# Emieeel/auto_oo

Measured on AMD Instinct MI355X. Metric: OO-VQE energy+grad evals/sec (formaldimine CAS(4e,3o)/cc-pVDZ); 2e-transform fp64 TFLOP/s vs roofline, higher is better.
Workload: dtype f64; 1 GPU; configs[1] shape: N=43 AOs, n_occ=6, CAS(4e,3o), UCCD n_theta=4, n_kappa=327; one step = one batched call evaluating energy + full gradient of all 256 geometries of the rank (256 synthetic geometries in the job, geometry g on rank g mod n_gpus); value = evaluations/s; in-order calls on one stream; geometries_per_rank=256, batched_calls=1332, calls=in order, parallelism=geometry-sharded x1, one all_gather at the end, dist_world_size=1, devices_visible=1, device_of_rank0=0

## Files before the change

### auto_oo_amd/csrc/api.hip

```cpp
#include "common.h"
#include <stdarg.h>
#include <vector>
#include <utility>

static thread_local char g_err[512] = "";

void oovqe_set_error(const char* fmt, ...)
{
    va_list ap;
    va_start(ap, fmt);
    vsnprintf(g_err, sizeof(g_err), fmt, ap);
    va_end(ap);
}

extern "C" int oovqe_version(void) { return 100; }

extern "C" const char* oovqe_last_error(void) { return g_err; }

extern "C" int oovqe_device_count(void)
{
    int n = 0;
    hipError_t e = hipGetDeviceCount(&n);
    if (e != hipSuccess) {
        oovqe_set_error("hipGetDeviceCount: %s", hipGetErrorString(e));
        return -1;
    }
    return n;
}

#include <mutex>
#include <map>
int oovqe_ensure_dynamic_lds(const void* kernel, size_t bytes)
{
    static std::mutex mu;
    static std::map<std::pair<const void*, int>, size_t> done;
    int dev = 0;
    if (hipGetDevice(&dev) != hipSuccess) dev = 0;
    std::lock_guard<std::mutex> lock(mu);
    size_t& have = done[std::make_pair(kernel, dev)];
    if (bytes <= have) return 0;
    hipError_t e = hipFuncSetAttribute(kernel, hipFuncAttributeMaxDynamicSharedMemorySize, (int)bytes);
    if (e != hipSuccess) {
        oovqe_set_error("hipFuncSetAttribute(MaxDynamicSharedMemorySize = %zu): %s", bytes, hipGetErrorString(e));
        return OOVQE_ERR_HIP;
    }
    have = bytes;
    return 0;
}

static int g_opts[OOVQE_OPT_COUNT] = {0};
static const char* const g_opt_names[OOVQE_OPT_COUNT] = {
    "half_stream_old", "gm_two_per_cu", "gm_one_per_cu", "fused_chunks", "tri_plain_w", "cas_unfused",
    "sym_no_rs", "sym_mirror", "sym_simple", "sym_two_step", "no_ride", "tri_mode", "k1_no_pair", "k1_force_wide", "gm_plain_grid",
    "newton_one_wg", "sector_unfused", "sector_probe", "hess_vk_pass", "hess_own_stage1", "panel_rows",
    "k1_force_nt", "newton_no_chol", "tiles_variant", "sector_lambda_w", "sector_rdm_r3", "gm_three_per_cu", "panel_no_w",
    "stage1_free_run", "one_stream"};
static_assert(sizeof(g_opt_names) / sizeof(g_opt_names[0]) == OOVQE_OPT_COUNT, "option name table out of step with oovqe_option_t");

int oovqe_opt(int id) { return (id >= 0 && id < OOVQE_OPT_COUNT) ? g_opts[id] : 0; }

static char g_stage1[160] = "";
void oovqe_note_stage1(const char* fmt, ...)
{
    va_list ap;
    va_start(ap, fmt);
    vsnprintf(g_stage1, sizeof(g_stage1), fmt, ap);
    va_end(ap);
}
extern "C" const char* oovqe_last_stage1_kernel(void) { return g_stage1; }

extern "C" int oovqe_debug_set_option(const char* name, int value)
{
    for (int i = 0; name && i < OOVQE_OPT_COUNT; ++i)
        if (strcmp(name, g_opt_names[i]) == 0) { g_opts[i] = value; return 0; }
    oovqe_set_error("oovqe_debug_set_option: unknown option '%s'", name ? name : "(null)");
    return OOVQE_ERR_ARG;
}

extern "C" int oovqe_debug_get_option(const char* name)
{
    for (int i = 0; name && i < OOVQE_OPT_COUNT; ++i)
        if (strcmp(name, g_opt_names[i]) == 0) return g_opts[i];
    return -1;
}

namespace {
struct Internals {
    hipEvent_t ev[64] = {};
    hipStream_t st[1] = {nullptr};
    unsigned next = 0;
    bool tried = false, streams_tried = false;
};
Internals g_int[16];
std::mutex g_int_mu;

Internals* internals()
{
    int dev = 0;
    if (hipGetDevice(&dev) != hipSuccess || dev < 0 || dev >= 16) return nullptr;
    Internals& I = g_int[dev];
    if (!I.tried) {
        I.tried = true;
        for (int i = 0; i < 64; ++i)
            if (hipEventCreateWithFlags(&I.ev[i], hipEventDisableTiming) != hipSuccess) I.ev[i] = nullptr;
    }
    return &I;
}
}

hipEvent_t oovqe_internal_event()
{
    std::lock_guard<std::mutex> lock(g_int_mu);
    Internals* I = internals();
    return I ? I->ev[I->next++ & 63] : nullptr;
}

hipStream_t oovqe_internal_stream(int k)
{
    if (oovqe_opt(OOVQE_OPT_ONE_STREAM) != 0 || k != 0) return nullptr;
    std::lock_guard<std::mutex> lock(g_int_mu);
    Internals* I = internals();
    if (!I) return nullptr;
    if (!I->streams_tried) {
        I->streams_tried = true;
        if (hipStreamCreateWithFlags(&I->st[0], hipStreamNonBlocking) != hipSuccess) I->st[0] = nullptr;
    }
    return I->st[k];
}

static hipStream_t g_s1_stream[16];
static hipEvent_t g_s1_event[16];
static bool g_s1_seen[16];
static int g_s1_multi[16];

int oovqe_stage1_enter(hipStream_t st)
{
    int dev = 0;
    if (hipGetDevice(&dev) != hipSuccess || dev < 0 || dev >= 16) return 0;
    if (oovqe_opt(OOVQE_OPT_STAGE1_FREE_RUN) != 0) return 0;
// ... 123 lines not shown
```

### auto_oo_amd/csrc/cas.hip

```cpp
#include "common.h"
#include "circuit_small.h"
#include <type_traits>
#include <stdlib.h>

int oovqe_mode_contract_impl(const double* T, const double* Cm, double* out, long A, int K, int J,
                             long B, int ldc, int last, hipStream_t st);
int oovqe_mode_contract_batched(const double* T, const double* Cm, double* out, long A, int K, int J,
                                long B, int ldc, int last, int batch, long t_bs, long c_bs, long o_bs,
                                hipStream_t st);
int oovqe_mode_contract_batched_circ(const double* T, const double* Cm, double* out, long A, int K, int J,
                                     long B, int ldc, int last, int batch, long t_bs, long c_bs,
                                     long o_bs, hipStream_t st, const oovqe_circuit_job_t* cj);
int oovqe_contract_hosts_circuit(long A, int K, int J, long B, int last, int batch);
int oovqe_circuit_rdms_w(const double* theta, int n_theta, const oovqe_gate_t* gates, int n_gates, int n_qubits,
                         int ncas, uint32_t init_index, int want_tangents, int batch, double* psi, double* dpsi,
                         double* gamma, double* Gamma, double* work, const double* h_ao, const double* C, int N,
                         double* Wpre, oovqe_stream_t stream);
extern "C" int oovqe_circuit_rdms(const double* theta, int n_theta, const oovqe_gate_t* gates, int n_gates,
                                  int n_qubits, int ncas, uint32_t init_index, int want_tangents, int batch,
                                  double* psi, double* dpsi, double* gamma, double* Gamma, double* work,
                                  oovqe_stream_t stream);
extern "C" int oovqe_circuit_rdms_is_small(int n_qubits, int ncas, int nvec, int n_gates);

namespace {
// ... 2655 lines not shown
    }
    for (int o = 32; o > 0; o >>= 1) part += __shfl_xor(part, o);
    if ((tid & 63) == 0) red[tid >> 6] = part;
    __syncthreads();
    if (tid == 0) Epart[(size_t)k * N + n] = (red[0] + red[1]) + (red[2] + red[3]);
    if (k == 0) {
        if (tid == 0) Cpart[n] = n < no ? hmo[(size_t)n * M + n] + FIn[n] : 0.0;
        if (n >= no && n < M) {
            const int p = n - no;
            for (int q = tid; q < na; q += FROW_THREADS) c1[p * na + q] = FIn[no + q];
            for (int idx = tid; idx < na3; idx += FROW_THREADS) c2[(size_t)p * na3 + idx] = 0.5 * cube[idx];
        }
    }
}

__global__ __launch_bounds__(512)
void cas_final_kernel(const double* __restrict__ Fcol, const double* __restrict__ Epart,
                      const double* __restrict__ Cpart, double nuc, int nrdm, int N, int M,
                      const int32_t* __restrict__ kap_row, const int32_t* __restrict__ kap_col,
                      int n_kappa, double* __restrict__ c0, double* __restrict__ E,
                      double* __restrict__ gvec, double* __restrict__ dE, double* __restrict__ fock,
                      double* __restrict__ gmat, const double* __restrict__ nuc_arr,
                      size_t out_stride)
{
    const int tid = threadIdx.x;
    {
        const size_t gi = blockIdx.x;
        Fcol += gi * (size_t)nrdm * M * N;
        Epart += gi * (size_t)nrdm * N;
        Cpart += gi * (size_t)N;
        c0 += gi * out_stride;
        E += gi * out_stride;
        gvec += gi * out_stride;
        if (dE) dE += gi * out_stride;
        if (fock) fock += gi * (size_t)N * N;
        if (gmat) gmat += gi * (size_t)N * N;
        if (nuc_arr) nuc = nuc_arr[gi];
    }
    for (long base = 0; base < (long)nrdm * n_kappa; base += 4 * 512) {
        int rr[4], cc[4], kk[4];
#pragma unroll
        for (int u = 0; u < 4; ++u) {
            const long idx = base + u * 512 + tid;
            const bool ok = idx < (long)nrdm * n_kappa;
            const long ii = ok ? idx : 0;
            kk[u] = (int)(ii / n_kappa);
            const int t = (int)(ii - (long)kk[u] * n_kappa);
            rr[u] = kap_row[t];
            cc[u] = kap_col[t];
        }
        double frc[4], fcr[4];
#pragma unroll
        for (int u = 0; u < 4; ++u) {
            const double* F = Fcol + (size_t)kk[u] * M * N;
            const int r = rr[u], c = cc[u];
            frc[u] = F[(size_t)(r < M ? r : 0) * N + c] * (r < M ? 1.0 : 0.0);
            fcr[u] = F[(size_t)(c < M ? c : 0) * N + r] * (c < M ? 1.0 : 0.0);
        }
#pragma unroll
        for (int u = 0; u < 4; ++u) {
            const long idx = base + u * 512 + tid;
            if (idx < (long)nrdm * n_kappa) gvec[idx] = 2.0 * (frc[u] - fcr[u]);
        }
    }
    if (fock)
        for (int idx = tid; idx < N * N; idx += 512) {
            const int m = idx / N;
            fock[idx] = m < M ? Fcol[idx] : 0.0;
        }
    if (gmat)
        for (int idx = tid; idx < N * N; idx += 512) {
            const int m = idx / N, n = idx - m * N;
            const double fmn = m < M ? Fcol[(size_t)m * N + n] : 0.0;
            const double fnm = n < M ? Fcol[(size_t)n * N + m] : 0.0;
            gmat[idx] = 2.0 * (fmn - fnm);
        }
    if (tid < nrdm) {
        const int k = tid;
        double acc = 0.0;
        for (int n = 0; n < M; ++n) acc += Epart[(size_t)k * N + n];
        if (k == 0) {
            double core = nuc;
            for (int n = 0; n < M; ++n) core += Cpart[n];
            c0[0] = core;
            E[0] = core + acc;
        } else if (dE) {
            dE[k - 1] = acc;
        }
    }
}

}

static int half_transform_batched(const double* g_ao, const double* C, int N, int M, double* T2,
                                  int batch, oovqe_stream_t stream, int sym = SYM_FULL, bool rs = false,
                                  double* Vk_tri = nullptr, const double* g_tiles = nullptr);
static int device_cu_count();

extern "C" int oovqe_cas_half_transform(const double* g_ao, const double* C, int N, int M, double* T2,
                                        oovqe_stream_t stream)
{
    return half_transform_batched(g_ao, C, N, M, T2, 1, stream);
}

static int half_transform_batched(const double* g_ao, const double* C, int N, int M, double* T2,
                                  int batch, oovqe_stream_t stream, int sym, bool rs, double* Vk_tri,
                                  const double* g_tiles)
{
    OOVQE_REQUIRE(g_ao && C && T2, "cas_half_transform: null pointer");
    OOVQE_REQUIRE(!Vk_tri || (sym == SYM_MIRROR && N <= 48),
                  "cas_half_transform: the quarter-transformed output needs p<->q symmetric integrals and N <= 48");
    OOVQE_REQUIRE(batch >= 1 && batch <= 65535, "cas_half_transform: batch=%d", batch);
    OOVQE_REQUIRE(N >= 1 && M >= 1 && M <= N, "cas_half_transform: bad N=%d M=%d", N, M);
    hipStream_t st = (hipStream_t)stream;
    const int ZT = (M + 15) / 16;
    const int nrb = (N + 15) / 16;
    const int ksteps = (N + 3) / 4;
    const int LDM = 16 * (ZT | 1);
    const size_t lds_elems = (((size_t)nrb * 16 * LDM + 511) / 512) * 512;
    const size_t lds_bytes = lds_elems * sizeof(double);
    OOVQE_REQUIRE(ZT <= 3, "cas_half_transform: n_occ+ncas = %d > 48 not supported", M);
    OOVQE_REQUIRE(lds_bytes <= 160 * 1024, "cas_half_transform: N=%d M=%d needs %zu B of LDS", N, M,
                  lds_bytes);
    const long nslabs = sym == SYM_FULL ? (long)N * N : (long)N * (N + 1) / 2;
    int kch = ksteps <= 4 ? 4 : ksteps <= 8 ? 8 : ksteps <= 11 ? 11 : ksteps <= 12 ? 12 : 16;
    const int nkc = (ksteps + kch - 1) / kch;
#define OOVQE_LAUNCH_HALF(Z, KC_, NS_)                                                            \
    do {                                                                                          \
        static bool attr_done = false;                                                            \
        if (!attr_done) {                                                                         \
            hipError_t e = hipFuncSetAttribute((const void*)half_transform_kernel<Z, KC_, NS_>,   \
                                               hipFuncAttributeMaxDynamicSharedMemorySize,        \
                                               160 * 1024);                                       \
            if (e != hipSuccess) {                                                                \
                oovqe_set_error("cas_half_transform: hipFuncSetAttribute: %s",                    \
                                hipGetErrorString(e));                                            \
                return OOVQE_ERR_HIP;                                                             \
            }                                                                                     \
            attr_done = true;                                                                     \
        }                                                                                         \
        oovqe_note_stage1("half_transform_kernel<%d,%d,%d>%s", Z, KC_, NS_, sym ? " (slabs p <= q)" : ""); \
        const unsigned wpg = (NS_) > 0 ? 4u : (unsigned)HALF_WAVES;             \
        hipLaunchKernelGGL((half_transform_kernel<Z, KC_, NS_>),                                  \
                           dim3((unsigned)((nslabs + wpg - 1) / wpg), batch), dim3(wpg * 64),     \
                           (NS_) > 0 ? 0 : lds_bytes, st, g_ao, C, T2, N, M, nrb, nkc, nslabs, sym, Vk_tri); \
    } while (0)
#define OOVQE_DISPATCH_KCH(Z)                                                                     \
    do {                                                                                          \
              \
        if (kch == 4 && nrb == 1) OOVQE_LAUNCH_HALF(Z, 4, 1);                                     \
        else if (kch == 8 && nrb == 2) OOVQE_LAUNCH_HALF(Z, 8, 2);                                \
        else if (kch == 11 && nrb == 3) OOVQE_LAUNCH_HALF(Z, 11, 3);                              \
        else if (kch == 12 && nrb == 3) OOVQE_LAUNCH_HALF(Z, 12, 3);                              \
        else OOVQE_LAUNCH_HALF(Z, 16, 0);                           \
    } while (0)
    const bool stream_old = oovqe_opt(OOVQE_OPT_HALF_STREAM_OLD) != 0;
    if (nrb > 3 && !stream_old) {
        int skch = 16, waste = 1 << 30;
        for (int k = 16; k >= 10; --k) {
            const int w = (ksteps + k - 1) / k * k - ksteps;
            if (w < waste) { waste = w; skch = k; }
        }
        const int snkc = (ksteps + skch - 1) / skch;
        const long want = (nslabs + HALF_WAVES - 1) / HALF_WAVES;
        const size_t lds_rs = lds_bytes + (size_t)HALF_WAVES * 16 * 17 * sizeof(double);
        const bool use_rs = rs && lds_rs <= 160 * 1024;
// ... 139 lines not shown
    int* bad = (int*)malloc(sizeof(int) * (size_t)batch);
    if (!bad) e = hipErrorOutOfMemory;
    if (e == hipSuccess) e = hipMemcpyAsync(bad, flag, sizeof(int) * (size_t)batch, hipMemcpyDeviceToHost, st);
    if (e == hipSuccess) e = hipStreamSynchronize(st);
    (void)hipFree(flag);
    if (e == hipSuccess)
        for (int gi = 0; gi < batch; ++gi)
            eri_flags[gi] = ((bad[gi] & 1) ? 0u : OOVQE_ERI_PQ_SYMMETRIC) | ((bad[gi] & 2) ? 0u : OOVQE_ERI_RS_SYMMETRIC);
    free(bad);
    OOVQE_CHECK_HIP(e, "eri_ingest");
    return 0;
}

static int sym_q_contract_batched(const double* J, const double* C, double* T3, int N, int M, int batch,
                                  hipStream_t st)
{
    OOVQE_REQUIRE(M >= 1 && M <= 16 && N >= 1 && N <= 48, "sym_q_contract: N=%d M=%d", N, M);
    const unsigned threads = (unsigned)((M * M + 15) / 16 * 64);
    const int ksteps = (N + 3) / 4;
    oovqe_profile_mark_start_l(st, 5);
    if (ksteps <= 4)
        hipLaunchKernelGGL(sym_q_contract_kernel<4>, dim3(N, batch), dim3(threads), 0, st, J, C, T3, N, M);
    else if (ksteps <= 8)
        hipLaunchKernelGGL(sym_q_contract_kernel<8>, dim3(N, batch), dim3(threads), 0, st, J, C, T3, N, M);
    else
        hipLaunchKernelGGL(sym_q_contract_kernel<12>, dim3(N, batch), dim3(threads), 0, st, J, C, T3, N, M);
    oovqe_profile_mark_stop(st);
    OOVQE_CHECK_LAUNCH("cas_eval/sym_q_contract");
    return 0;
}

static int sym_gm_batched(const double* J, const double* C, double* Gm, int N, int M, int batch,
                          hipStream_t st, const oovqe_circuit_job_t* cj, bool packed)
{
    OOVQE_REQUIRE(M >= 1 && M <= 16 && N >= 1 && N <= 48, "sym_gm: N=%d M=%d", N, M);
    const int ksteps = (N + 3) / 4;
    int KSr = ksteps <= 4 ? 4 : ksteps <= 8 ? 8 : 12;
    size_t lds_bytes = (size_t)4 * KSr * (M * 16 + 8) * sizeof(double);
    if (cj && cj->lds_bytes > lds_bytes) lds_bytes = cj->lds_bytes;
    const size_t lds11 = (size_t)44 * (M * 16 + 8) * sizeof(double);
    const bool three_per_cu = ksteps == 11 && (!cj || cj->lds_bytes <= lds11) && 3 * lds11 <= 160 * 1024 &&
                              oovqe_opt(OOVQE_OPT_GM_THREE_PER_CU) == 1;
    const unsigned nty = (unsigned)(((packed ? M * (M + 1) / 2 : M * M) + 15) / 16);
    oovqe_circuit_job_t job;
    memset(&job, 0, sizeof(job));
    if (cj) job = *cj;
    const unsigned nx = nty + (cj ? 1 : 0);
    const bool xcd_grid = batch > 1 && oovqe_opt(OOVQE_OPT_GM_PLAIN_GRID) == 0;
    const dim3 grid = xcd_grid ? dim3(nx * (unsigned)((batch + 7) / 8 * 8)) : dim3(nx, batch);
#define OOVQE_LAUNCH_GM2(KS_, WPE_)                                                               \
    do {                                                                                          \
        static size_t attr_bytes = 0;                                                             \
        if (lds_bytes > attr_bytes) {                                                             \
            OOVQE_CHECK_HIP(hipFuncSetAttribute((const void*)sym_gm_kernel<KS_, WPE_>,            \
                                                hipFuncAttributeMaxDynamicSharedMemorySize,       \
                                                (int)lds_bytes), "cas_eval/sym_gm");              \
            attr_bytes = lds_bytes;                                                               \
        }                                                                                         \
        hipLaunchKernelGGL((sym_gm_kernel<KS_, WPE_>), grid, dim3(SMALL_THREADS), lds_bytes, st,  \
                           J, C, Gm, N, M, packed ? 1 : 0, job, cj ? 1 : 0, batch);               \
    } while (0)
    const bool multi_round = ((long)(nty + (cj ? 1 : 0)) * batch > (long)device_cu_count() || oovqe_opt(OOVQE_OPT_GM_TWO_PER_CU)) &&
                             2 * lds_bytes <= 160 * 1024 && oovqe_opt(OOVQE_OPT_GM_ONE_PER_CU) == 0;
#define OOVQE_LAUNCH_GM(KS_)                                                                      \
    do {                                                                                          \
        if (multi_round) OOVQE_LAUNCH_GM2(KS_, 4);                                                \
        else OOVQE_LAUNCH_GM2(KS_, 2);                                                            \
    } while (0)
    oovqe_profile_mark_start_l(st, 2);
    if (three_per_cu) {
        KSr = 11;
        lds_bytes = lds11;
        OOVQE_LAUNCH_GM2(11, 6);
    } else if (KSr == 4) OOVQE_LAUNCH_GM(4);
    else if (KSr == 8) OOVQE_LAUNCH_GM(8);
    else OOVQE_LAUNCH_GM(12);
    oovqe_profile_mark_stop(st);
#undef OOVQE_LAUNCH_GM
#undef OOVQE_LAUNCH_GM2
    OOVQE_CHECK_LAUNCH("cas_eval/sym_gm");
    return 0;
}

struct FusedPlan {
    int nchunk, qc, nbuf, ldb, wpg;
    size_t lds_bytes;
};

static int device_cu_count()
{
    static int n_cu = 0;
    if (!n_cu) {
        int dev = 0;
        hipDeviceProp_t prop;
        if (hipGetDevice(&dev) == hipSuccess && hipGetDeviceProperties(&prop, dev) == hipSuccess)
            n_cu = prop.multiProcessorCount;
        if (n_cu <= 0) n_cu = 256;
    }
    return n_cu;
}

static bool fused_plan(int N, int M, int batch, FusedPlan* fp)
{
    if (M > 16 || N > 48 || N < 1) return false;
    const long chunks_env = oovqe_opt(OOVQE_OPT_FUSED_CHUNKS);
    const long m2 = (long)M * M, m3 = m2 * M;
    const int n_cu = device_cu_count();
    if (chunks_env <= 0 && (long)batch * N * N < 48L * n_cu) return false;
    long target = n_cu / batch;
    long nchunk0 = chunks_env > 0 ? chunks_env : target / N;
    if (nchunk0 < 1) nchunk0 = 1;
    const long cap = (2L * N * m2 - m3) / (m3 + N);
    if (cap < 1) return false;
    if (nchunk0 > cap) nchunk0 = cap;
    int qc = N, nchunk = 1;
    if (nchunk0 > 1) {
        qc = 4 * (int)((N + 4 * nchunk0 - 1) / (4 * nchunk0));
        nchunk = (N + qc - 1) / qc;
    }
    const int QR = (qc + 3) & ~3, CR = (nchunk - 1) * qc + QR;
    int ldb = (int)((m2 + 15) / 16 * 16);
    if (ldb % 32 == 0) ldb += 16;
    const size_t fixed = ((size_t)CR * 16 + 64 + 8) * sizeof(double);
    const size_t block = (size_t)QR * ldb * sizeof(double);
    const size_t task_stage = (size_t)m3 * sizeof(double);
    const long Tg = (long)nchunk * N;
    long wpg = target < 1 ? 1 : target;
    if (wpg > Tg) wpg = Tg;
    const size_t lds_cap = 160 * 1024;
    if (fixed + 2 * block + task_stage > lds_cap) return false;
    const long max_tasks = (long)((lds_cap - fixed - 2 * block) / task_stage);
    if ((Tg + wpg - 1) / wpg > max_tasks) wpg = (Tg + max_tasks - 1) / max_tasks;
    const long ntask = (Tg + wpg - 1) / wpg;
    long nbuf = (long)((lds_cap - fixed - (size_t)ntask * task_stage) / block);
    if (nbuf > 3) nbuf = 3;
    fp->nchunk = nchunk;
    fp->qc = qc;
    fp->nbuf = (int)nbuf;
    fp->ldb = ldb;
    fp->wpg = (int)wpg;
    fp->lds_bytes = fixed + (size_t)nbuf * block + (size_t)ntask * task_stage;
    return true;
}

static int half_transform_fused_batched(const double* g_ao, const double* C, int N, int M, double* T3,
                                        double* Cdup, const FusedPlan& fp, int batch, hipStream_t st)
{
    const int ksteps = (N + 3) / 4, nrb = (N + 15) / 16;
    const int kch = ksteps <= 4 ? 4 : ksteps <= 8 ? 8 : ksteps <= 11 ? 11 : 12;
#define OOVQE_LAUNCH_FUSED(KC_, NS_)                                                              \
    do {                                                                                          \
        static bool attr_done = false;                                                            \
        if (!attr_done) {                                                                         \
            hipError_t e = hipFuncSetAttribute((const void*)half_transform_fused_kernel<KC_, NS_>, \
                                               hipFuncAttributeMaxDynamicSharedMemorySize,        \
                                               160 * 1024);                                       \
            if (e != hipSuccess) {                                                                \
                oovqe_set_error("cas_eval: hipFuncSetAttribute: %s", hipGetErrorString(e));       \
                return OOVQE_ERR_HIP;                                                             \
            }                                                                                     \
            attr_done = true;                                                                     \
        }                                                                                         \
        oovqe_note_stage1("half_transform_fused_kernel<%d,%d>", KC_, NS_);                        \
        hipLaunchKernelGGL((half_transform_fused_kernel<KC_, NS_>), dim3(fp.wpg, batch),          \
                           dim3(HALF_WAVES * 64), fp.lds_bytes, st, g_ao, C, T3, Cdup, N, M,      \
                           fp.nchunk, fp.qc, fp.nbuf, fp.ldb);                                    \
// ... 319 lines not shown
{
    const size_t na2 = (size_t)ncas * ncas;
    return column_base_bytes(N, M) + (na2 + na2 * na2) * sizeof(double) <= 160 * 1024;
}

extern "C" int64_t oovqe_oo_eval_out_size(int n_theta, int n_kappa, int ncas, int derivatives);

static bool cas_w_block(int N, int M, int batch, unsigned eri_flags, double* work, double** W)
{
    if (N > 48 || oovqe_opt(OOVQE_OPT_CAS_UNFUSED) != 0 || oovqe_opt(OOVQE_OPT_SYM_MIRROR) != 0 ||
        oovqe_opt(OOVQE_OPT_SYM_SIMPLE) != 0 || oovqe_opt(OOVQE_OPT_SYM_TWO_STEP) != 0 ||
        oovqe_opt(OOVQE_OPT_PANEL_NO_W) != 0 || (eri_flags & OOVQE_ERI_PQ_SYMMETRIC) == 0)
        return false;
    FusedPlan fp;
    if (!fused_plan(N, M, batch, &fp)) return false;
    const long m2 = (long)M * M, m3 = m2 * M;
    const long tri = (long)N * (N + 1) / 2;
    const long nty16 = (m2 + 15) / 16 * 16;
    if (tri * nty16 + 2 * (long)N * m3 > 2 * (long)N * N * m2) return false;
    *W = work + (size_t)batch * tri * nty16;
    return true;
}

static int cas_eval_batched(const double* g_ao, const double* h_ao, const double* C,
                            const double* gamma, const double* Gamma, int nrdm, double nuc,
                            const double* nuc_arr, int N, int n_occ, int ncas, const int32_t* kap_row,
                            const int32_t* kap_col, int n_kappa, double* work, double* c0, double* c1,
                            double* c2, double* E, double* gvec, double* dE, double* fock,
                            double* gmat, double* Gm, double* hmo, int batch, size_t out_stride,
                            oovqe_stream_t stream, const oovqe_circuit_job_t* cj = nullptr,
                            unsigned eri_flags = 0, const double* g_packed = nullptr,
                            const double* T2_ready = nullptr, bool w_ready = false, hipEvent_t rdm_event = nullptr)
{
    OOVQE_REQUIRE(g_ao && h_ao && C && gamma && Gamma && work && c0 && c1 && c2 && E && gvec,
                  "cas_eval: null pointer");
    OOVQE_REQUIRE(nrdm >= 1 && N >= 1 && n_occ >= 0 && ncas >= 1 && n_occ + ncas <= N,
                  "cas_eval: bad sizes");
    OOVQE_REQUIRE(n_kappa == 0 || (kap_row && kap_col), "cas_eval: null index table");
    OOVQE_REQUIRE(nrdm == 1 || dE, "cas_eval: dE required when nrdm > 1");
    OOVQE_REQUIRE(batch >= 1 && batch <= 65535, "cas_eval: batch=%d", batch);
    hipStream_t st = (hipStream_t)stream;
    const int M = n_occ + ncas;
    const long m2 = (long)M * M, m3 = m2 * M;
    const size_t nb = (size_t)batch;
    double* T2 = work;
    double* U = T2 + nb * N * N * m2;
    double* Fcol = U + nb * N * N * m2;
    double* Epart = Fcol + nb * nrdm * M * N;
    double* Cpart = Epart + nb * nrdm * N;
    int rc;
    const bool unfused_env = oovqe_opt(OOVQE_OPT_CAS_UNFUSED) != 0;
    FusedPlan fp;
    const bool fused = !unfused_env && fused_plan(N, M, batch, &fp);
    const double* Gm_in = nullptr;
    const double* Wpre = nullptr;
    const bool pq_sym = (eri_flags & OOVQE_ERI_PQ_SYMMETRIC) != 0;
    const bool rs_sym = (eri_flags & OOVQE_ERI_RS_SYMMETRIC) != 0 && oovqe_opt(OOVQE_OPT_SYM_NO_RS) == 0;
    const int half_sym = pq_sym ? SYM_MIRROR : SYM_FULL;
    const long tri = (long)N * (N + 1) / 2;
    const long nty16 = (m2 + 15) / 16 * 16;
    const bool sym_packed = fused && pq_sym && oovqe_opt(OOVQE_OPT_SYM_MIRROR) == 0 &&
                            tri * nty16 + 2 * (long)N * m3 <= 2 * (long)N * N * m2;
    if (sym_packed) {
        double* Jp = work;
        double* T3 = Jp + nb * tri * nty16;
        double* Gmw = T3 + nb * N * m3;
        const bool simple = oovqe_opt(OOVQE_OPT_SYM_SIMPLE) != 0;
        const bool two_step = simple || oovqe_opt(OOVQE_OPT_SYM_TWO_STEP) != 0;
        if (simple) {
            if ((rc = half_transform_batched(g_ao, C, N, M, Jp, batch, stream, SYM_PACKED))) return rc;
        } else {
            const bool use_pk = !two_step && rs_sym && g_packed != nullptr;
            if (T2_ready && !two_step) {
                const unsigned nbk = (unsigned)((tri + 15) / 16);
                oovqe_profile_mark_start_l(st, 0);
                hipLaunchKernelGGL(j_from_t2_kernel, dim3(nbk, batch), dim3(256), 0, st, T2_ready, Jp, N, M,
                                   rs_sym ? 1 : 0);
                oovqe_profile_mark_stop(st);
                OOVQE_CHECK_LAUNCH("cas_eval/j_from_t2");
            } else if ((rc = half_tri_batched(use_pk ? g_packed : g_ao, C, N, M, Jp, batch, st,
                                              two_step ? 0 : rs_sym ? 2 : 1, use_pk)))
                return rc;
        }
        if (!two_step) {
            if ((rc = sym_gm_batched(Jp, C, Gmw, N, M, batch, st, cj, rs_sym))) return rc;
            if (rdm_event && cj) {
                OOVQE_CHECK_HIP(hipEventRecord(rdm_event, st), "cas_eval: hipEventRecord");
                rdm_event = nullptr;
            }
            if (w_ready) {
                double* wchk = nullptr;
                OOVQE_REQUIRE(cas_w_block(N, M, batch, eri_flags, work, &wchk) && wchk == T3,
                              "cas_eval: W = C^T h was promised for another path");
                Wpre = T3;
            }
        } else {
            if ((rc = sym_q_contract_batched(Jp, C, T3, N, M, batch, st))) return rc;
            oovqe_profile_mark_start_l(st, 2);
            if ((rc = oovqe_mode_contract_batched_circ(T3, C, Gmw, 1, N, N, m3, N, 0, batch, (long)N * m3,
                                                       (long)N * N, (long)N * m3, st, cj)))
                return rc;
            oovqe_profile_mark_stop(st);
        }
        Gm_in = Gmw;
    } else if (fused) {
        double* T3 = work;
        double* Gmw = T3 + nb * fp.nchunk * N * m3;
        double* Cdup = Gmw + nb * N * m3;
        if ((rc = half_transform_fused_batched(g_ao, C, N, M, T3, Cdup, fp, batch, st))) return rc;
        oovqe_profile_mark_start_l(st, 2);
        const long K = (long)fp.nchunk * N;
        if ((rc = oovqe_mode_contract_batched_circ(T3, fp.nchunk > 1 ? Cdup : C, Gmw, 1, (int)K, N, m3, N, 0,
                                                   batch, K * m3, fp.nchunk > 1 ? K * N : (long)N * N,
                                                   (long)N * m3, st, cj)))
            return rc;
        oovqe_profile_mark_stop(st);
        Gm_in = Gmw;
    } else if (!column_fits(N, M, ncas)) {
        OOVQE_REQUIRE(M < N, "cas_eval: the staged path needs at least one virtual orbital (N=%d M=%d)", N, M);
        if (cj) {
            if ((rc = oovqe_circuit_rdms(cj->theta, cj->n_theta, cj->gates, cj->n_gates, cj->n_qubits,
                                         cj->ncas, cj->init_index, cj->n_tan > 0, batch, nullptr, nullptr,
                                         cj->gamma, cj->Gamma, nullptr, stream)))
                return rc;
        }
        if ((rc = half_transform_batched(g_ao, C, N, M, T2, batch, stream, half_sym, rs_sym, nullptr,
                                         N > 48 ? g_packed : nullptr)))
            return rc;
        const size_t na2s = (size_t)ncas * ncas, na4s = na2s * na2s;
        for (int g = 0; g < batch; ++g) {
            const size_t gi = (size_t)g;
            double* T2g = T2 + gi * N * N * m2;
            double* wk = U + gi * N * N * m2;
            double* Gmg = T2g;
            double* hmog = Fcol + gi * nrdm * M * N;
            if ((rc = oovqe_cas_finish_transform(T2g, h_ao + gi * N * N, C + gi * N * N, N, M, Gmg, hmog,
                                                 wk, stream)))
                return rc;
            double* Fc = wk + (size_t)N * m3 + (size_t)N * M;
            double* Ep = Fc + (size_t)nrdm * M * N;
            double* Cp = Ep + (size_t)nrdm * N;
            const bool rows_fit = (size_t)N * m3 + (size_t)N * M + (size_t)nrdm * (M + 1) * N + N <=
                                  (size_t)N * N * m2 && M <= 64 &&
                                  fock_rows_lds_elems(n_occ, ncas) * sizeof(double) <= FROW_LDS_MAX;
            if (rows_fit)
                rc = cas_energy_gradient_rows(
                    Gmg, hmog, gamma + gi * nrdm * na2s, Gamma + gi * nrdm * na4s, nrdm, nuc,
                    nuc_arr ? nuc_arr + g : nullptr, N, n_occ, ncas, kap_row, kap_col, n_kappa, Fc, Ep, Cp,
                    c0 + gi * out_stride, c1 + gi * out_stride, c2 + gi * out_stride, E + gi * out_stride,
                    fock ? fock + gi * N * N : nullptr, gmat ? gmat + gi * N * N : nullptr,
                    gvec + gi * out_stride, dE ? dE + gi * out_stride : nullptr, stream);
            else
                rc = cas_energy_gradient_impl(
                    Gmg, hmog, gamma + gi * nrdm * na2s, Gamma + gi * nrdm * na4s, nrdm, nuc,
                    nuc_arr ? nuc_arr + g : nullptr, N, n_occ, ncas, kap_row, kap_col, n_kappa,
                    c0 + gi * out_stride, c1 + gi * out_stride, c2 + gi * out_stride, E + gi * out_stride,
                    fock ? fock + gi * N * N : nullptr, gmat ? gmat + gi * N * N : nullptr,
                    gvec + gi * out_stride, dE ? dE + gi * out_stride : nullptr, stream);
            if (rc) return rc;
            if (Gm)
                OOVQE_CHECK_HIP(hipMemcpyAsync(Gm + gi * N * m3, Gmg, (size_t)N * m3 * sizeof(double),
                                               hipMemcpyDeviceToDevice, st), "cas_eval: copy g_mo");
            if (hmo)
                OOVQE_CHECK_HIP(hipMemcpyAsync(hmo + gi * N * M, hmog, (size_t)N * M * sizeof(double),
                                               hipMemcpyDeviceToDevice, st), "cas_eval: copy h_mo");
        }
// ... 345 lines not shown
```

### auto_oo_amd/csrc/common.h

```cpp
#pragma once
#include <hip/hip_runtime.h>
#include <stdint.h>
#include <stdio.h>
#include <string.h>
#include "../../include/oovqe.h"

typedef double d4 __attribute__((ext_vector_type(4)));
typedef double d2 __attribute__((ext_vector_type(2)));
typedef double d2u __attribute__((ext_vector_type(2), aligned(8)));

#define OOVQE_ERR_ARG   (-1)
#define OOVQE_ERR_HIP   (-2)
#define OOVQE_ERR_SIZE  (-3)

void oovqe_set_error(const char* fmt, ...);
void oovqe_profile_mark_start(hipStream_t st);
void oovqe_profile_mark_start_l(hipStream_t st, int label);
void oovqe_profile_mark_stop(hipStream_t st);

enum oovqe_option_t {
    OOVQE_OPT_HALF_STREAM_OLD = 0,
    OOVQE_OPT_GM_TWO_PER_CU,
    OOVQE_OPT_GM_ONE_PER_CU,
    OOVQE_OPT_FUSED_CHUNKS,
    OOVQE_OPT_TRI_PLAIN_W,
    OOVQE_OPT_CAS_UNFUSED,
    OOVQE_OPT_SYM_NO_RS,
    OOVQE_OPT_SYM_MIRROR,
    OOVQE_OPT_SYM_SIMPLE,
    OOVQE_OPT_SYM_TWO_STEP,
    OOVQE_OPT_NO_RIDE,
    OOVQE_OPT_TRI_MODE,
    OOVQE_OPT_K1_NO_PAIR,
    OOVQE_OPT_K1_FORCE_WIDE,
    OOVQE_OPT_GM_PLAIN_GRID,
    OOVQE_OPT_NEWTON_ONE_WG,
    OOVQE_OPT_SECTOR_UNFUSED,
    OOVQE_OPT_SECTOR_PROBE,
    OOVQE_OPT_HESS_VK_PASS,
    OOVQE_OPT_HESS_OWN_STAGE1,
    OOVQE_OPT_PANEL_ROWS,
    OOVQE_OPT_K1_FORCE_NT,
    OOVQE_OPT_NEWTON_NO_CHOL,
    OOVQE_OPT_TILES_VARIANT,
    OOVQE_OPT_SECTOR_LAMBDA_W,
    OOVQE_OPT_SECTOR_RDM_R3,
    OOVQE_OPT_GM_THREE_PER_CU,
    OOVQE_OPT_PANEL_NO_W,
    OOVQE_OPT_STAGE1_FREE_RUN,
    OOVQE_OPT_ONE_STREAM,
    OOVQE_OPT_COUNT
};
int oovqe_opt(int id);
int oovqe_ensure_dynamic_lds(const void* kernel, size_t bytes);
void oovqe_note_stage1(const char* fmt, ...);
hipEvent_t oovqe_internal_event();
hipStream_t oovqe_internal_stream(int k);
int oovqe_stage1_enter(hipStream_t st);
int oovqe_stage1_leave(hipStream_t st);

#define OOVQE_CHECK_LAUNCH(name)                                                          \
    do {                                                                                  \
        hipError_t e__ = hipGetLastError();                                               \
        if (e__ != hipSuccess) {                                                          \
            oovqe_set_error("%s: launch failed: %s", name, hipGetErrorString(e__));       \
            return OOVQE_ERR_HIP;                                                         \
        }                                                                                 \
    } while (0)

#define OOVQE_CHECK_HIP(call, name)                                                        \
    do {                                                                                  \
        hipError_t e__ = (call);                                                          \
        if (e__ != hipSuccess) {                                                          \
            oovqe_set_error("%s: %s", name, hipGetErrorString(e__));                      \
            return OOVQE_ERR_HIP;                                                         \
        }                                                                                 \
    } while (0)

#define OOVQE_REQUIRE(cond, ...)                                                          \
    do {                                                                                  \
        if (!(cond)) {                                                                    \
            oovqe_set_error(__VA_ARGS__);                                                 \
            return OOVQE_ERR_ARG;                                                         \
        }                                                                                 \
    } while (0)

struct oovqe_circuit_job_t {
    const double* theta;
    const oovqe_gate_t* gates;
    double* gamma;
    double* Gamma;
    int n_theta, n_gates, n_qubits, ncas, n_tan, count;
    uint32_t init_index;
    size_t lds_bytes;
};

__device__ __forceinline__ d4 mfma_f64(double a, double b, d4 c) {
    return __builtin_amdgcn_mfma_f64_16x16x4f64(a, b, c, 0, 0, 0);
}


__device__ __forceinline__ long clamp_u32(long rem)
{
    int hi = (int)(rem >> 32);
    const unsigned lo = (unsigned)rem;
    asm("" : "+s"(hi));
    return (long)(hi < 0 ? 0u : (hi != 0 ? 0xFFFFFFFFu : lo));
}
```

Measured before the change: 554,500 evals/s.

## Fuse second-stage transform and gradient tail into one per-geometry kernel

Adds a cas_tail_kernel that runs one workgroup per geometry. It does the second half-transform of the two-electron integrals with MFMA, keeps in LDS only the (x,y,z) index columns the gradient actually needs, then computes the inactive Fock matrix, the generalized Fock rows, the energy and the orbital gradient in the same kernel. This replaces the separate sym_gm pass and the follow-on kernels, removing their launches and global round-trips. The path is on by default when the batch exceeds twice the CU count and the LDS budget fits; a tail_split option restores the old path. The tradeoff is lower parallelism per geometry, with much serial scalar work inside each block.

```diff
diff --git a/auto_oo_amd/csrc/api.hip b/auto_oo_amd/csrc/api.hip
--- a/auto_oo_amd/csrc/api.hip
+++ b/auto_oo_amd/csrc/api.hip
@@ -54,7 +54,7 @@
     "sym_no_rs", "sym_mirror", "sym_simple", "sym_two_step", "no_ride", "tri_mode", "k1_no_pair", "k1_force_wide", "gm_plain_grid",
     "newton_one_wg", "sector_unfused", "sector_probe", "hess_vk_pass", "hess_own_stage1", "panel_rows",
     "k1_force_nt", "newton_no_chol", "tiles_variant", "sector_lambda_w", "sector_rdm_r3", "gm_three_per_cu", "panel_no_w",
-    "stage1_free_run", "one_stream"};
+    "stage1_free_run", "one_stream", "tail_split"};
 static_assert(sizeof(g_opt_names) / sizeof(g_opt_names[0]) == OOVQE_OPT_COUNT, "option name table out of step with oovqe_option_t");
 
 int oovqe_opt(int id) { return (id >= 0 && id < OOVQE_OPT_COUNT) ? g_opts[id] : 0; }
diff --git a/auto_oo_amd/csrc/cas.hip b/auto_oo_amd/csrc/cas.hip
--- a/auto_oo_amd/csrc/cas.hip
+++ b/auto_oo_amd/csrc/cas.hip
@@ -2761,6 +2761,335 @@
         if (k == 0) {
             double core = nuc;
             for (int n = 0; n < M; ++n) core += Cpart[n];
+            c0[0] = core;
+            E[0] = core + acc;
+        } else if (dE) {
+            dE[k - 1] = acc;
+        }
+    }
+}
+
+constexpr int TAIL_THREADS = 512;
+
+__host__ __device__ inline bool tail_needed(int x, int y, int z, int no)
+{
+    const int lo = y < z ? y : z, hi = y < z ? z : y;
+    if (lo >= no) return true;
+    if (hi < no) return lo == hi || x == lo || x == hi;
+    return x >= no || x == lo;
+}
+
+template <int KS>
+__global__ __launch_bounds__(TAIL_THREADS, 2)
+void cas_tail_kernel(const double* __restrict__ J, const double* __restrict__ C, const double* __restrict__ Wpre,
+                     const double* __restrict__ gamma, const double* __restrict__ Gamma, int nrdm, int N, int no,
+                     int na, int NC, double nuc, const double* __restrict__ nuc_arr,
+                     const int32_t* __restrict__ kap_row, const int32_t* __restrict__ kap_col, int n_kappa,
+                     double* __restrict__ c0, double* __restrict__ E, double* __restrict__ gvec,
+                     double* __restrict__ dE, double* __restrict__ c1, double* __restrict__ c2, size_t out_stride)
+{
+    extern __shared__ double lds[];
+    constexpr int NW = TAIL_THREADS / 64;
+    constexpr int PW = (4 * KS + NW - 1) / NW;
+    constexpr int PB = PW * KS > 48 ? (PW + 1) / 2 : PW;
+    const int M = no + na, M2 = M * M, M3 = M2 * M;
+    const int na2 = na * na, na3 = na2 * na, na4 = na2 * na2;
+    const int ncol = M * (M + 1) / 2, nty = (ncol + 15) / 16;
+    const long tri = (long)N * (N + 1) / 2;
+    const int by = blockIdx.x;
+    const int tid = threadIdx.x, lane = tid & 63;
+    const int wave = __builtin_amdgcn_readfirstlane(tid >> 6);
+    const int lq = lane >> 4, lr = lane & 15;
+    {
+        const size_t gi = by;
+        J += gi * nty * tri * 16;
+        C += gi * (size_t)N * N;
+        Wpre += gi * (size_t)N * N;
+        gamma += gi * (size_t)nrdm * na2;
+        Gamma += gi * (size_t)nrdm * na4;
+        c0 += gi * out_stride;
+        E += gi * out_stride;
+        gvec += gi * out_stride;
+        if (dE) dE += gi * out_stride;
+        c1 += gi * out_stride;
+        c2 += gi * out_stride;
+        if (nuc_arr) nuc = nuc_arr[gi];
+    }
+    double* Gc = lds;
+    double* Cl = Gc + (size_t)N * NC;
+    double* hn = Cl + (size_t)N * M;
+    double* FIn = hn + (size_t)N * M;
+    double* gml = FIn + (size_t)N * M;
+    double* Gml = gml + (size_t)nrdm * na2;
+    double* Cp = Gml + (size_t)nrdm * na4;
+    int* tab = reinterpret_cast<int*>(Cp + N);
+    int* wcnt = tab + M3;
+    int* krow = wcnt + NW;
+    int* kcol = krow + n_kappa;
+    double* scr = Cp + N + (M3 + NW + 2 * n_kappa + 1) / 2;
+    const int LDP = M * 16 + 8;
+
+    typedef unsigned v2u __attribute__((ext_vector_type(2)));
+    const __amdgpu_buffer_rsrc_t csrd = __builtin_amdgcn_make_buffer_rsrc(
+        const_cast<double*>(C), 0, (int)((size_t)N * N * sizeof(double)), 0x00020000);
+    double af[KS];
+#pragma unroll
+    for (int ks = 0; ks < KS; ++ks) {
+        const int q = 4 * ks + lq;
+        const v2u v = __builtin_amdgcn_raw_buffer_load_b64(
+            csrd, (q < N && lr < M) ? (unsigned)((q * N + lr) * (int)sizeof(double)) : 0x7fffffffu, 0, 0);
+        af[ks] = __builtin_bit_cast(double, v);
+    }
+    auto load_half = [&](double (&bf)[PB][KS], int ty, int h0) {
+        const __amdgpu_buffer_rsrc_t jsrd = __builtin_amdgcn_make_buffer_rsrc(
+            const_cast<double*>(J + (size_t)ty * tri * 16), 0, (int)(tri * 16 * sizeof(double)), 0x00020000);
+#pragma unroll
+        for (int i = 0; i < PB; ++i) {
+            const int p = wave + NW * (h0 + i);
+            const int pc = p < N ? p : N - 1;
+            const int basep = pc * (2 * N - pc + 1) / 2 - pc;
+#pragma unroll
+            for (int ks = 0; ks < KS; ++ks) {
+                const int q = 4 * ks + lq < N ? 4 * ks + lq : N - 1;
+                const int t = q < pc ? q * (2 * N - q + 1) / 2 - q + pc : basep + q;
+                const v2u v = __builtin_amdgcn_raw_buffer_load_b64(
+                    jsrd, (unsigned)((t * 16 + lr) * (int)sizeof(double)), 0, 0);
+                bf[i][ks] = __builtin_bit_cast(double, v);
+            }
+        }
+    };
+    double* T3s = scr;
+    auto mfma_half = [&](const double (&bf)[PB][KS], int h0) {
+#pragma unroll
+        for (int i = 0; i < PB; ++i) {
+            if (h0 + i >= PW) continue;
+            const int p = wave + NW * (h0 + i);
+            d4 acc = d4{0.0, 0.0, 0.0, 0.0};
+#pragma unroll
+            for (int ks = 0; ks < KS; ++ks) acc = mfma_f64(af[ks], bf[i][ks], acc);
+            double* row = T3s + (size_t)(p < 4 * KS ? p : 0) * LDP + lr;
+#pragma unroll
+            for (int j = 0; j < 4; ++j) {
+                const int x = lq + 4 * j;
+                if (x < M && p < 4 * KS) row[x * 16] = p < N ? acc[j] : 0.0;
+            }
+        }
+    };
+    static_assert(2 * PB >= PW, "two halves cover the rows of a wave");
+    double bf[PB][KS];
+    load_half(bf, 0, 0);
+
+    for (int idx = tid; idx < N * M; idx += TAIL_THREADS) {
+        const int q = idx / M, x = idx - q * M;
+        Cl[idx] = C[(size_t)q * N + x];
+    }
+    for (int idx = tid; idx < N * N; idx += TAIL_THREADS) scr[idx] = Wpre[idx];
+    for (int idx = tid; idx < nrdm * na2; idx += TAIL_THREADS) gml[idx] = gamma[idx];
+    for (int idx = tid; idx < nrdm * na4; idx += TAIL_THREADS) Gml[idx] = Gamma[idx];
+    for (int idx = tid; idx < n_kappa; idx += TAIL_THREADS) {
+        krow[idx] = kap_row[idx];
+        kcol[idx] = kap_col[idx];
+    }
+    {
+        const int total = M * ncol;
+        int base = 0;
+        for (int i0 = 0; i0 < total; i0 += TAIL_THREADS) {
+            const int i = i0 + tid;
+            int x = 0, y = 0, z = 0;
+            bool need = false;
+            if (i < total) {
+                x = i / ncol;
+                tri_decode(i - x * ncol, M, y, z);
+                need = tail_needed(x, y, z, no);
+            }
+            const unsigned long long mask = __ballot(need);
+            const int below = __popcll(mask & ((1ull << lane) - 1ull));
+            if (lane == 0) wcnt[wave] = __popcll(mask);
+            __syncthreads();
+            int pre = base, all = 0;
+            for (int w = 0; w < NW; ++w) {
+                const int c = wcnt[w];
+                if (w < wave) pre += c;
+                all += c;
+            }
+            if (i < total) {
+                const int v = need ? pre + below : -1;
+                tab[(x * M + y) * M + z] = v;
+                tab[(x * M + z) * M + y] = v;
+            }
+            __syncthreads();
+            base += all;
+        }
+    }
+    for (int idx = tid; idx < N * M; idx += TAIL_THREADS) {
+        const int n = idx / M, x = idx - n * M;
+        double acc = 0.0;
+        for (int q = 0; q < N; ++q) acc += scr[(size_t)n * N + q] * Cl[q * M + x];
+        hn[idx] = acc;
+    }
+    __syncthreads();
+
+    {
+        const int ntn = (N + 15) / 16;
+        for (int ty = 0; ty < nty; ++ty) {
+            mfma_half(bf, 0);
+            if (PB < PW) {
+                load_half(bf, ty, PB);
+                mfma_half(bf, PB);
+            }
+            __syncthreads();
+            const int yz = 16 * ty + lr;
+            int off = 0;
+            if (yz < ncol) {
+                int y, z;
+                tri_decode(yz, M, y, z);
+                off = y * M + z;
+            }
+            int cur_nt = -1;
+            double cf[KS];
+            for (int tile = wave; tile < ntn * M; tile += NW) {
+                const int nt = tile / M, x = tile - nt * M;
+                if (nt != cur_nt) {
+                    const int n = 16 * nt + lr;
+#pragma unroll
+                    for (int ks = 0; ks < KS; ++ks) {
+                        const int pp = 4 * ks + lq;
+                        const v2u v = __builtin_amdgcn_raw_buffer_load_b64(
+                            csrd, (pp < N && n < N) ? (unsigned)((pp * N + n) * (int)sizeof(double)) : 0x7fffffffu,
+                            0, 0);
+                        cf[ks] = __builtin_bit_cast(double, v);
+                    }
+                    cur_nt = nt;
+                }
+                double tf[KS];
+#pragma unroll
+                for (int ks = 0; ks < KS; ++ks) tf[ks] = T3s[(size_t)(4 * ks + lq) * LDP + x * 16 + lr];
+                d4 acc = d4{0.0, 0.0, 0.0, 0.0};
+#pragma unroll
+                for (int ks = 0; ks < KS; ++ks) acc = mfma_f64(cf[ks], tf[ks], acc);
+                const int ci = yz < ncol ? tab[x * M2 + off] : -1;
+                if (ci >= 0) {
+#pragma unroll
+                    for (int j = 0; j < 4; ++j) {
+                        const int n = 16 * nt + lq + 4 * j;
+                        if (n < N) Gc[(size_t)n * NC + ci] = acc[j];
+                    }
+                }
+            }
+            if (ty + 1 < nty) load_half(bf, ty + 1, 0);
+            __syncthreads();
+        }
+    }
+
+#define TAIL_G(n, a, b, c) Gc[(size_t)(n) * NC + tab[((a) * M + (b)) * M + (c)]]
+    for (int idx = tid; idx < N * M; idx += TAIL_THREADS) {
+        const int n = idx / M, x = idx - n * M;
+        double fi = hn[idx];
+        for (int i = 0; i < no; ++i) fi += 2.0 * TAIL_G(n, x, i, i) - TAIL_G(n, i, i, x);
+        FIn[idx] = fi;
+    }
+    double* Fl = scr;
+    double* El = Fl + (size_t)nrdm * M * N;
+    double* Ga = El + (size_t)nrdm * N;
+    double* Dc = Ga + (size_t)N * na3;
+    for (int idx = tid; idx < N * na3; idx += TAIL_THREADS) {
+        const int n = idx / na3, r = idx - n * na3;
+        const int w = r / na2, x = (r / na) % na, y = r % na;
+        Ga[idx] = TAIL_G(n, no + w, no + x, no + y);
+    }
+    for (int idx = tid; idx < N * no * na2; idx += TAIL_THREADS) {
+        const int n = idx / (no * na2), r = idx - n * (no * na2);
+        const int m = r / na2, v = (r / na) % na, w = r % na;
+        const int V = no + v, W = no + w;
+        Dc[idx] = TAIL_G(n, m, V, W) - 0.5 * TAIL_G(n, W, V, m);
+    }
+    __syncthreads();
+    for (int n = tid; n < N; n += TAIL_THREADS) Cp[n] = n < no ? hn[n * M + n] + FIn[n * M + n] : 0.0;
+    for (int idx = tid; idx < na * (na + na3); idx += TAIL_THREADS) {
+        const int pl = idx / (na + na3), r0 = idx - pl * (na + na3);
+        const int n = no + pl;
+        if (r0 < na) {
+            c1[pl * na + r0] = FIn[n * M + no + r0];
+        } else {
+            int t = r0 - na;
+            const int i3 = t;
+            const int s = t % na; t /= na;
+            const int r = t % na; t /= na;
+            const int q = t;
+            c2[(size_t)pl * na3 + i3] = 0.5 * TAIL_G(n, no + q, no + r, no + s);
+        }
+    }
+    const int ncore = N * nrdm * no;
+    for (int idx = tid; idx < N * nrdm * M; idx += TAIL_THREADS) {
+        int n, k, m;
+        if (idx < ncore) {
+            n = idx / (nrdm * no);
+            const int r0 = idx - n * (nrdm * no);
+            k = r0 / no;
+            m = r0 - k * no;
+        } else {
+            const int j = idx - ncore;
+            n = j / (nrdm * na);
+            const int r0 = j - n * (nrdm * na);
+            k = r0 / na;
+            m = no + r0 - k * na;
+        }
+        const double* FIv = FIn + (size_t)n * M;
+        const double* gam = gml + (size_t)k * na2;
+        double val;
+        if (m < no) {
+            const double* Dm = Dc + ((size_t)n * no + m) * na2;
+            double fa = 0.0;
+            for (int v = 0; v < na; ++v)
+                for (int w = 0; w < na; ++w) fa += gam[v * na + w] * Dm[v * na + w];
+            val = 2.0 * ((k == 0 ? FIv[m] : 0.0) + fa);
+        } else {
+            const int v = m - no;
+            const double* Gv = Gml + (size_t)k * na4 + (size_t)v * na3;
+            double acc = 0.0;
+            for (int w = 0; w < na; ++w) acc += FIv[no + w] * gam[v * na + w];
+            for (int w = 0; w < na; ++w)
+                for (int x = 0; x < na; ++x)
+                    for (int y = 0; y < na; ++y)
+                        acc += Gv[(w * na + x) * na + y] * Ga[(size_t)n * na3 + (w * na + x) * na + y];
+            val = acc;
+        }
+        Fl[((size_t)k * M + m) * N + n] = val;
+    }
+    for (int idx = tid; idx < N * nrdm; idx += TAIL_THREADS) {
+        const int n = idx / nrdm, k = idx - n * nrdm;
+        double acc = 0.0;
+        if (n >= no && n < M) {
+            const int p = n - no;
+            const double* FIv = FIn + (size_t)n * M;
+            const double* gam = gml + (size_t)k * na2 + (size_t)p * na;
+            const double* Gpq = Gml + (size_t)k * na4 + (size_t)p * na3;
+            for (int q = 0; q < na; ++q) acc += FIv[no + q] * gam[q];
+            for (int q = 0; q < na; ++q)
+                for (int r = 0; r < na; ++r)
+                    for (int s2 = 0; s2 < na; ++s2)
+                        acc += 0.5 * Ga[(size_t)n * na3 + (q * na + r) * na + s2] * Gpq[(q * na + r) * na + s2];
+        }
+        El[(size_t)k * N + n] = acc;
+    }
+#undef TAIL_G
+    __syncthreads();
+
+    for (int idx = tid; idx < nrdm * n_kappa; idx += TAIL_THREADS) {
+        const int k = idx / n_kappa, t = idx - k * n_kappa;
+        const int r = krow[t], c = kcol[t];
+        const double* F = Fl + (size_t)k * M * N;
+        const double frc = F[(size_t)(r < M ? r : 0) * N + c] * (r < M ? 1.0 : 0.0);
+        const double fcr = F[(size_t)(c < M ? c : 0) * N + r] * (c < M ? 1.0 : 0.0);
+        gvec[idx] = 2.0 * (frc - fcr);
+    }
+    if (tid < nrdm) {
+        const int k = tid;
+        double acc = 0.0;
+        for (int n = 0; n < M; ++n) acc += El[(size_t)k * N + n];
+        if (k == 0) {
+            double core = nuc;
+            for (int n = 0; n < M; ++n) core += Cp[n];
             c0[0] = core;
             E[0] = core + acc;
         } else if (dE) {
@@ -3066,6 +3395,62 @@
     return 0;
 }
 
+static size_t tail_lds_bytes(int N, int no, int na, int nrdm, int n_kappa, int* NC)
+{
+    const int M = no + na, M3 = M * M * M;
+    if (N > 48 || M > 16) return 0;
+    int nc = 0;
+    for (int x = 0; x < M; ++x)
+        for (int y = 0; y < M; ++y)
+            for (int z = y; z < M; ++z) nc += tail_needed(x, y, z, no) ? 1 : 0;
+    *NC = nc;
+    const int ksteps = (N + 3) / 4, KSr = ksteps <= 4 ? 4 : ksteps <= 8 ? 8 : 12;
+    const size_t na2 = (size_t)na * na, na4 = na2 * na2;
+    size_t scr = (size_t)N * N;
+    const size_t t3 = (size_t)4 * KSr * (M * 16 + 8);
+    const size_t fe = (size_t)nrdm * M * N + (size_t)nrdm * N +
+                      (size_t)N * na * na * na + (size_t)N * no * na2;
+    if (t3 > scr) scr = t3;
+    if (fe > scr) scr = fe;
+    const size_t doubles = (size_t)N * nc + 3 * (size_t)N * M + (size_t)nrdm * (na2 + na4) + N +
+                           ((size_t)M3 + TAIL_THREADS / 64 + 2 * (size_t)n_kappa + 1) / 2 + scr;
+    const size_t bytes = doubles * sizeof(double);
+    return bytes <= 160 * 1024 ? bytes : 0;
+}
+
+static int cas_tail_batched(const double* J, const double* C, const double* Wpre, const double* gamma,
+                            const double* Gamma, int nrdm, double nuc, const double* nuc_arr, int N, int n_occ,
+                            int ncas, const int32_t* kap_row, const int32_t* kap_col, int n_kappa, double* c0,
+                            double* c1, double* c2, double* E, double* gvec, double* dE, int batch,
+                            size_t out_stride, hipStream_t st)
+{
+    int NC = 0;
+    const size_t lds_bytes = tail_lds_bytes(N, n_occ, ncas, nrdm, n_kappa, &NC);
+    OOVQE_REQUIRE(lds_bytes > 0, "cas_eval/tail: N=%d M=%d nrdm=%d does not fit", N, n_occ + ncas, nrdm);
+    const int ksteps = (N + 3) / 4;
+#define OOVQE_LAUNCH_TAIL(KS_)                                                                    \
+    do {                                                                                          \
+        static size_t attr_bytes = 0;                                                             \
+        if (lds_bytes > attr_bytes) {                                                             \
+            OOVQE_CHECK_HIP(hipFuncSetAttribute((const void*)cas_tail_kernel<KS_>,                \
+                                                hipFuncAttributeMaxDynamicSharedMemorySize,       \
+                                                (int)lds_bytes), "cas_eval/tail");                \
+            attr_bytes = lds_bytes;                                                               \
+        }                                                                                         \
+        hipLaunchKernelGGL((cas_tail_kernel<KS_>), dim3(batch), dim3(TAIL_THREADS), lds_bytes, st, J, C, Wpre, \
+                           gamma, Gamma, nrdm, N, n_occ, ncas, NC, nuc, nuc_arr, kap_row, kap_col, n_kappa, c0, \
+                           E, gvec, dE, c1, c2, out_stride);                                      \
+    } while (0)
+    oovqe_profile_mark_start_l(st, 2);
+    if (ksteps <= 4) OOVQE_LAUNCH_TAIL(4);
+    else if (ksteps <= 8) OOVQE_LAUNCH_TAIL(8);
+    else OOVQE_LAUNCH_TAIL(12);
+    oovqe_profile_mark_stop(st);
+#undef OOVQE_LAUNCH_TAIL
+    OOVQE_CHECK_LAUNCH("cas_eval/tail");
+    return 0;
+}
+
 struct FusedPlan {
     int nchunk, qc, nbuf, ldb, wpg;
     size_t lds_bytes;
@@ -3551,6 +3936,20 @@
                                               two_step ? 0 : rs_sym ? 2 : 1, use_pk)))
                 return rc;
         }
+        int tail_nc = 0;
+        const bool tail = !two_step && rs_sym && g_packed != nullptr && !T2_ready && !cj && w_ready && !fock && !gmat && !Gm && !hmo &&
+                          2L * batch > (long)device_cu_count() && tail_lds_bytes(N, n_occ, ncas, nrdm, n_kappa, &tail_nc) > 0 &&
+                          oovqe_opt(OOVQE_OPT_TAIL_SPLIT) == 0;
+        if (tail) {
+            double* wchk = nullptr;
+            OOVQE_REQUIRE(cas_w_block(N, M, batch, eri_flags, work, &wchk) && wchk == T3,
+                          "cas_eval: W = C^T h was promised for another path");
+            if ((rc = cas_tail_batched(Jp, C, T3, gamma, Gamma, nrdm, nuc, nuc_arr, N, n_occ, ncas, kap_row, kap_col,
+                                       n_kappa, c0, c1, c2, E, gvec, dE, batch, out_stride, st)))
+                return rc;
+            if (rdm_event) OOVQE_CHECK_HIP(hipEventRecord(rdm_event, st), "cas_eval: hipEventRecord");
+            return 0;
+        }
         if (!two_step) {
             if ((rc = sym_gm_batched(Jp, C, Gmw, N, M, batch, st, cj, rs_sym))) return rc;
             if (rdm_event && cj) {
diff --git a/auto_oo_amd/csrc/common.h b/auto_oo_amd/csrc/common.h
--- a/auto_oo_amd/csrc/common.h
+++ b/auto_oo_amd/csrc/common.h
@@ -49,6 +49,7 @@
     OOVQE_OPT_PANEL_NO_W,
     OOVQE_OPT_STAGE1_FREE_RUN,
     OOVQE_OPT_ONE_STREAM,
+    OOVQE_OPT_TAIL_SPLIT,
     OOVQE_OPT_COUNT
 };
 int oovqe_opt(int id);
```

New measurement: 576,200 evals/s (median of 6 runs). 1.04x the previous value.
